# KubiakJakub01/Blokus-RL

Measured on AMD Instinct MI355X. Metric: MCTS sims/sec on 20x20 Blokus (4 players, 256 games/GPU, 100 sims/move), higher is better.
Workload: dtype fp32 net (fp32 operands split into f16 hi+lo, 3 f16 MFMA products, f32 accumulation: fp32-class error, tests/test_leafnet_gpu.py) / f64 search / u32 bitboards; 1 GPU; config 3 (N=1) / 4 (N=8): AlphaZero self-play 20x20, 256 concurrent games per GPU, 100 sims/move, ResNet-5x64 leaf eval; global_batch=256, parallelism=dp1 (independent games), model=resnet

## Files before the change

### blokus_rl_amd/csrc/leafnet.hip

```cpp
#include "../../include/blokus_engine.h"
#include "ctx.h"

#include <type_traits>

#define BK_LN_VACC 1
#include "leafnet_common.h"

#ifndef BK_LN_EPIW
#define BK_LN_EPIW 1
#endif

namespace bk {
namespace {

constexpr bool kLnEpiWrite = BK_LN_EPIW != 0;
#ifndef BK_LN_IL
#define BK_LN_IL 1
#endif
constexpr bool kLnInterleave = BK_LN_IL != 0;

struct LnStates {
  const uint32_t* states;
  const int32_t* status;
};
constexpr int kLnP = kStemCinX3 / 2;
constexpr int kLnRowWords = kLnP * kMaxN;

template <int N, typename In>
__global__ __launch_bounds__(kLnThreads, 1) void k_leafnet_x3(In in,
                                                              const h16x8* __restrict__ wstem_a,
                                                              const float* __restrict__ sstem_a,
                                                              const float* __restrict__ bstem_a,
                                                              const h16x8* __restrict__ wt_a,
                                                              const float* __restrict__ st_a,
                                                              const float* __restrict__ bt_a,
                                                              const float* __restrict__ bounds_a, int nlayers,
                                                              LnHeads hd_a, float* __restrict__ xout) {
  constexpr bool ROWS = std::is_same<In, LnRows>::value;
  constexpr bool STATES = std::is_same<In, LnStates>::value || ROWS;
  const h16x8* __restrict__ wstem = wstem_a;
  const float* __restrict__ sstem = sstem_a;
  const float* __restrict__ bstem = bstem_a;
  const h16x8* __restrict__ wt = wt_a;
  const float* __restrict__ st = st_a;
  const float* __restrict__ bt = bt_a;
  const float* __restrict__ bounds = bounds_a;
  LnHeads hd = hd_a;
  size_t b = blockIdx.x;
  if constexpr (ROWS) {
    int k;
    const int t = ln_row_tree(in, blockIdx.x, k);
    if (t < 0) return;
    b = (size_t)t;
    const LnNet nk = ln_pick(in.nets, k);
    wstem = nk.wstem;
    sstem = nk.sstem;
    bstem = nk.bstem;
    wt = nk.wt;
    st = nk.st;
    bt = nk.bt;
    bounds = nk.bounds;
    hd.wp = nk.wp;
    hd.bp = nk.bp;
    hd.wv = nk.wv;
    hd.bv = nk.bv;
    hd.w1t = nk.w1t;
    hd.b1 = nk.b1;
    hd.w2 = nk.w2;
    hd.b2 = nk.b2;
  }
  constexpr int NN = N * N, RS = ln_row(N), NG = ln_groups(N), PIX_IT = (NN + kLnThreads - 1) / kLnThreads;
  constexpr int PL = ln_plane(N);
  extern __shared__ __attribute__((aligned(16))) unsigned char lds[];
  unsigned char* act = lds;
  unsigned char* sin = lds + 16 * PL;
  float* red = reinterpret_cast<float*>(lds + ln_lds_body(N));
  constexpr int X0L = ln_x0_lds_groups(N);
  f32x4* x0s = reinterpret_cast<f32x4*>(lds + 16 * PL);
  const int tid = threadIdx.x, l = tid & 63, n = l & 15, ks = l >> 4;
  const int wave = __builtin_amdgcn_readfirstlane(tid >> 6);
  const int oc = 16 * wave + 4 * ks;
  LNSTAMP(0, __builtin_amdgcn_s_memtime());
  LNSTAMP(30, __builtin_amdgcn_s_memrealtime());

  float xin[STATES ? 1 : PIX_IT][kStemCinX3];
  uint32_t sw = 0u;
  bool live = true;
  if constexpr (STATES) {
    static_assert(kLnRowWords < kLnThreads && N <= kMaxN, "k_leafnet_x3: one state word per thread");
    live = ROWS || !in.status || in.status[b] == 1;
    if (live && tid <= kLnRowWords) sw = in.states[b * kStateWords + (tid < kLnRowWords ? tid : kWToMove)];
  } else {
    const float* __restrict__ ob = in + b * kStemCinX3 * NN;
#pragma unroll
    for (int it = 0; it < PIX_IT; ++it) {
      const int p = tid + it * kLnThreads;
#pragma unroll
      for (int c = 0; c < kStemCinX3; ++c) xin[it][c] = p < NN ? ob[c * NN + p] : 0.0f;
    }
  }
  {
    constexpr int kHaloCols = RS - N, kHalo = 2 * RS + N * kHaloCols;
    for (int i = tid; i < (STATES ? 17 : 18) * kHalo; i += kLnThreads) {
      const int plane = i / kHalo, k = i - plane * kHalo;
      int row, col;
      if (k < 2 * RS) {
        row = k < RS ? 0 : N + 1;
        col = k < RS ? k : k - RS;
      } else {
        const int h = k - 2 * RS, c = h % kHaloCols;
        row = 1 + h / kHaloCols;
        col = c == 0 ? 0 : N + c;
      }
      *reinterpret_cast<u32x4*>(lds + plane * PL + (row * RS + col) * 16) = u32x4{0u, 0u, 0u, 0u};
    }
  }

  constexpr int kBias = (RS + 1) * 16;
  int ab[NG];
  unsigned valid = 0;
#pragma unroll
  for (int g = 0; g < NG; ++g) {
    const int sl = kLnPixMap<N>.slot[16 * g + n];
    ab[g] = (sl >= 0 ? sl : RS + 1) * 16 + ks * 4 * PL - kBias;
    valid |= (sl >= 0 ? 1u : 0u) << g;
  }
  auto is_valid = [&](int g) { return NN % 16 == 0 || ((valid >> g) & 1u); };
  auto slot_b = [&](int g) { return ab[g] - ks * 4 * PL + kBias; };

  static_assert(18 % (kLnWpf + 1) == 0, "kLnWpf: the ring must divide the 18 chunks of a layer");
  constexpr int kLayerBlocks = 18 * 4 * 2;
  const __amdgpu_buffer_rsrc_t wrs = ln_rsrc(wt, (unsigned)nlayers * kLayerBlocks * 1024u);
  auto wload = [&](int layer, int c, int p) {
    return __builtin_bit_cast(h16x8, __builtin_amdgcn_raw_buffer_load_b128(
                                         wrs, l * 16, ((layer * kLayerBlocks + c * 8 + wave * 2 + p) * 64) * 16, 0));
  };
  h16x8 wq[kLnWpf + 1][2];
#pragma unroll
  for (int c = 0; c < kLnWpf; ++c) {
    wq[c][0] = wload(0, c, 0);
    wq[c][1] = wload(0, c, 1);
  }
  h16x8 wsa[3][2];
#pragma unroll
  for (int j = 0; j < 3; ++j) {
    wsa[j][0] = wstem[((j * 4 + wave) * 2) * 64 + l];
    wsa[j][1] = wstem[((j * 4 + wave) * 2 + 1) * 64 + l];
  }
  const f32x4 s_stem = *reinterpret_cast<const f32x4*>(sstem + oc), b_stem = *reinterpret_cast<const f32x4*>(bstem + oc);

  float max_obs;
  int ex;
  if constexpr (STATES) {
    uint32_t* rows = reinterpret_cast<uint32_t*>(sin + PL);
    bool any = false;
    if (tid < kLnRowWords) {
      const uint32_t bits = tid % kMaxN < N ? sw & ((1u << N) - 1u) : 0u;
      rows[tid] = bits;
      any = bits != 0u;
    } else if (tid == kLnRowWords) {
      const uint32_t tm = live ? sw : ~0u;
      rows[kLnRowWords] = tm;
      any = tm < (uint32_t)kLnP;
    }
    max_obs = block_max(any ? 1.0f : 0.0f, red + 8, wave, l);
    ex = scale_exp(max_obs);
    const unsigned one = __builtin_bit_cast(unsigned short, (_Float16)ldexpf(1.0f, ex));
    const uint32_t tm = rows[kLnRowWords];
    const unsigned m01 = ((tm == 0u ? 1u : 0u) | (tm == 1u ? 0x10000u : 0u)) * one;
    const unsigned m23 = ((tm == 2u ? 1u : 0u) | (tm == 3u ? 0x10000u : 0u)) * one;
#pragma unroll
    for (int it = 0; it < PIX_IT; ++it) {
      const int p = tid + it * kLnThreads;
      if (p < NN) {
        const int r = p / N, c = p % N;
        unsigned bit[kLnP];
#pragma unroll
        for (int q = 0; q < kLnP; ++q) bit[q] = (rows[q * kMaxN + r] >> c) & 1u;
        const u32x4 hi{(bit[0] | (bit[1] << 16)) * one, (bit[2] | (bit[3] << 16)) * one, m01, m23};
        *reinterpret_cast<u32x4*>(sin + ((r + 1) * RS + c + 1) * 16) = hi;
      }
    }
  } else {
    float m = 0.0f;
#pragma unroll
    for (int it = 0; it < PIX_IT; ++it)
#pragma unroll
      for (int c = 0; c < kStemCinX3; ++c) m = fmaxf(m, fabsf(xin[it][c]));
    max_obs = block_max(m, red + 8, wave, l);
    ex = scale_exp(max_obs);
#pragma unroll
    for (int it = 0; it < PIX_IT; ++it) {
      const int p = tid + it * kLnThreads;
      if (p < NN) {
        unsigned h[4], o[4];
#pragma unroll
        for (int q = 0; q < 4; ++q) split2(ldexpf(xin[it][2 * q], ex), ldexpf(xin[it][2 * q + 1], ex), h[q], o[q]);
        const u32x4 hi{h[0], h[1], h[2], h[3]}, lo{o[0], o[1], o[2], o[3]};
        unsigned char* dst = sin + ((p / N + 1) * RS + p % N + 1) * 16;
        *reinterpret_cast<u32x4*>(dst) = hi;
        *reinterpret_cast<u32x4*>(dst + PL) = lo;
      }
    }
  }
  __syncthreads();
  LNSTAMP(1, __builtin_amdgcn_s_memtime());
// ... 53 lines not shown
        split2(y01.x, y01.y, h0, l0);
        split2(y23.x, y23.y, h1, l1);
        if (write) {
          if (is_valid(g)) {
            *reinterpret_cast<u32x2*>(wbase + slot_b(g)) = u32x2{h0, h1};
            *reinterpret_cast<u32x2*>(wbase + slot_b(g) + PL) = u32x2{l0, l1};
          }
        } else {
          acc[g] = f32x4{__builtin_bit_cast(float, h0), __builtin_bit_cast(float, h1), __builtin_bit_cast(float, l0),
                         __builtin_bit_cast(float, l1)};
        }
      } else {
        acc[g] = f32x4{y01.x, y01.y, y23.x, y23.y};
      }
    }
    return ldexpf(mx, -k);
  };
  auto write_act = [&]() {
    const int o = 2 * wave + (ks >> 1);
    unsigned char* base = act + ((o & 3) * 4 + (o >> 2) * 2) * PL + (ks & 1) * 8;
#pragma unroll
    for (int g = 0; g < NG; ++g) {
      const u32x4 w = __builtin_bit_cast(u32x4, acc[g]);
      if (is_valid(g)) {
        *reinterpret_cast<u32x2*>(base + slot_b(g)) = u32x2{w.x, w.y};
        *reinterpret_cast<u32x2*>(base + slot_b(g) + PL) = u32x2{w.z, w.w};
      }
    }
  };
  auto out_exp = [&](int conv, float max_in) { return scale_exp(bounds[2 * conv] * max_in + bounds[2 * conv + 1]); };
  auto post_max = [&](float mx, int par) {
    mx = wave_max_f(mx);
    if (l == 0) red[4 * par + wave] = mx;
  };
  auto board_max = [&](int par) {
    return fmaxf(fmaxf(red[4 * par], red[4 * par + 1]), fmaxf(red[4 * par + 2], red[4 * par + 3]));
  };

  f32x4 x0[NG];
  float max_in;
  {
    const int ex_out = out_exp(0, max_obs);
#pragma unroll
    for (int g = 0; g < NG; ++g) x0[g] = f32x4{0.f, 0.f, 0.f, 0.f};
    const float mx = epilogue(s_stem, b_stem, true, false, x0, false, 0);
#pragma unroll
    for (int g = 0; g < NG; ++g) x0[g] = acc[g];
    const float up = ldexpf(1.0f, ex_out);
#pragma unroll
    for (int g = 0; g < NG; ++g) {
      unsigned h0, h1, l0, l1;
      split2(x0[g][0] * up, x0[g][1] * up, h0, l0);
      split2(x0[g][2] * up, x0[g][3] * up, h1, l1);
      acc[g] = f32x4{__builtin_bit_cast(float, h0), __builtin_bit_cast(float, h1), __builtin_bit_cast(float, l0),
                     __builtin_bit_cast(float, l1)};
    }
#pragma unroll
    for (int g = X0L; g < NG; ++g) asm volatile("" : "+a"(x0[g]));
    post_max(mx, 0);
    __syncthreads();
    write_act();
#pragma unroll
    for (int g = 0; g < X0L; ++g) {
      x0s[g * kLnThreads + tid] = x0[g];
      x0[g] = f32x4{0.f, 0.f, 0.f, 0.f};
    }
    __syncthreads();
    max_in = board_max(0);
    ex = ex_out;
  }
  LNSTAMP(3, __builtin_amdgcn_s_memtime());

  for (int layer = 0; layer < nlayers; ++layer) {
    const bool more = layer + 1 < nlayers;
    const f32x4 sv = *reinterpret_cast<const f32x4*>(st + layer * 64 + oc);
    const f32x4 bv = *reinterpret_cast<const f32x4*>(bt + layer * 64 + oc);
    const float bnd_a = bounds[2 * (layer + 1)], bnd_b = bounds[2 * (layer + 1) + 1];
    auto coff_of = [&](int c) {
      const int t = c >> 1;
      return 2 * (c & 1) * PL + ((t / 3 - 1) * RS + (t % 3 - 1)) * 16 + kBias;
    };
    ln_prime<NG, PL>(rb, act, ab, coff_of(0));
    if (layer == 1) LNSTAMP(26, __builtin_amdgcn_s_memtime());
#pragma unroll
    for (int c = 0; c < 18; ++c) {
      if (layer == 1 && c == 1) LNSTAMP(27, __builtin_amdgcn_s_memtime());
      if (layer == 1 && c == 9) LNSTAMP(28, __builtin_amdgcn_s_memtime());
      const int cn = c + kLnWpf, sn = cn % (kLnWpf + 1);
      if (cn < 18) {
        wq[sn][0] = wload(layer, cn, 0);
        wq[sn][1] = wload(layer, cn, 1);
      } else {
        const int nl = more ? layer + 1 : layer;
        wq[sn][0] = wload(nl, cn - 18, 0);
        wq[sn][1] = wload(nl, cn - 18, 1);
      }
      const h16x8* w = wq[c % (kLnWpf + 1)];
      if constexpr (kLnInterleave) {
        if (c == 0)
          ln_chunk_il<NG, true, PL>(acc, w[0], w[1], act, ab, coff_of(0), coff_of(1), rb);
        else
          ln_chunk_il<NG, false, PL>(acc, w[0], w[1], act, ab, coff_of(c), coff_of(c + 1 < 18 ? c + 1 : c), rb);
      } else {
        if (c == 0)
          ln_chunk<NG, true, PL>(acc, w[0], w[1], act, ab, coff_of(0), coff_of(1), rb);
        else
          ln_chunk<NG, false, PL>(acc, w[0], w[1], act, ab, coff_of(c), coff_of(c + 1 < 18 ? c + 1 : c), rb);
      }
    }
    if constexpr (kLnInterleave) asm volatile("s_waitcnt lgkmcnt(0)" ::: "memory");
    ln_mfma_drain(acc);
    if (layer < 8) LNSTAMP(4 + 2 * layer, __builtin_amdgcn_s_memtime());
    const bool last = layer + 1 == nlayers;
#ifndef BK_LN_ABL
#define BK_LN_ABL 0
#endif
    if (!last && BK_LN_ABL != 0) {
      if constexpr ((BK_LN_ABL & 2) == 0) {
        const int ex_out = scale_exp(bnd_a * max_in + bnd_b);
        const float mx = epilogue(sv, bv, !(layer & 1), false, x0, true, ex_out);
        max_in = fmaxf(max_in, mx);
        ex = ex_out;
      }
    } else if (!last && kLnEpiWrite) {
      const int ex_out = scale_exp(bnd_a * max_in + bnd_b);
      if (layer == 1) LNSTAMP(21, __builtin_amdgcn_s_memtime());
      __syncthreads();
      if (layer == 1) LNSTAMP(22, __builtin_amdgcn_s_memtime());
      const float mx = epilogue(sv, bv, !(layer & 1), false, x0, true, ex_out, true);
      if (layer == 1) LNSTAMP(23, __builtin_amdgcn_s_memtime());
      post_max(mx, (layer + 1) & 1);
      if (layer == 1) LNSTAMP(24, __builtin_amdgcn_s_memtime());
      __syncthreads();
      if (layer == 1) LNSTAMP(25, __builtin_amdgcn_s_memtime());
      max_in = board_max((layer + 1) & 1);
      ex = ex_out;
    } else if (!last) {
      const int ex_out = scale_exp(bnd_a * max_in + bnd_b);
      const float mx = epilogue(sv, bv, !(layer & 1), false, x0, true, ex_out);
      if (layer == 1) LNSTAMP(21, __builtin_amdgcn_s_memtime());
      post_max(mx, (layer + 1) & 1);
      if (layer == 1) LNSTAMP(22, __builtin_amdgcn_s_memtime());
      __syncthreads();
      if (layer == 1) LNSTAMP(23, __builtin_amdgcn_s_memtime());
      write_act();
      if (layer == 1) LNSTAMP(24, __builtin_amdgcn_s_memtime());
      __syncthreads();
      if (layer == 1) LNSTAMP(25, __builtin_amdgcn_s_memtime());
      max_in = board_max((layer + 1) & 1);
      ex = ex_out;
    } else {
#pragma unroll
      for (int g = 0; g < X0L; ++g) x0[g] = x0s[g * kLnThreads + tid];
      epilogue(sv, bv, true, true, x0, false, 0);
    }
    if (layer < 8) LNSTAMP(5 + 2 * layer, __builtin_amdgcn_s_memtime());
  }

  if (xout) {
#pragma unroll
    for (int g = 0; g < NG; ++g)
      if (is_valid(g))
        *reinterpret_cast<f32x4*>(xout + (b * NN + ln_pixel<N>(slot_b(g) / 16)) * 64 + oc) = acc[g];
  }
  __syncthreads();
  float* hp = reinterpret_cast<float*>(act);
  {
    const f32x4 wp0 = *reinterpret_cast<const f32x4*>(hd.wp + oc);
    const f32x4 wp1 = *reinterpret_cast<const f32x4*>(hd.wp + 64 + oc);
    const f32x4 wvv = *reinterpret_cast<const f32x4*>(hd.wv + oc);
#pragma unroll
    for (int g = 0; g < NG; ++g) {
      const f32x4 y = acc[g];
      float d[3];
      const f32x4* w[3] = {&wp0, &wp1, &wvv};
#pragma unroll
      for (int k = 0; k < 3; ++k) {
        const float a = y.x * (*w[k]).x + y.y * (*w[k]).y + y.z * (*w[k]).z + y.w * (*w[k]).w;
        const auto s16 = __builtin_amdgcn_permlane16_swap(__float_as_uint(a), __float_as_uint(a), false, false);
        const float a16 = __uint_as_float(s16[0]) + __uint_as_float(s16[1]);
        const auto s32 = __builtin_amdgcn_permlane32_swap(__float_as_uint(a16), __float_as_uint(a16), false, false);
        d[k] = __uint_as_float(s32[0]) + __uint_as_float(s32[1]);
      }
      if (ks == 0 && is_valid(g)) {
        float* dst = hp + (ln_pixel<N>(slot_b(g) / 16) * 4 + wave) * 3;
        dst[0] = d[0];
        dst[1] = d[1];
        dst[2] = d[2];
      }
    }
  }
  __syncthreads();
  LNSTAMP(20, __builtin_amdgcn_s_memtime());
  float* vfeat = hp + NN * 12;
  float* part = vfeat + NN;
  const float bp0 = hd.bp[0], bp1 = hd.bp[1], bv0 = hd.bv[0];
  for (int i = tid; i < NN; i += kLnThreads) {
    const float* q = hp + i * 12;
    const float p0 = ((q[0] + q[3]) + q[6]) + q[9], p1 = ((q[1] + q[4]) + q[7]) + q[10],
                pv = ((q[2] + q[5]) + q[8]) + q[11];
    hd.pf[b * 2 * NN + i] = fmaxf(p0 + bp0, 0.0f);
    hd.pf[b * 2 * NN + NN + i] = fmaxf(p1 + bp1, 0.0f);
    vfeat[i] = fmaxf(pv + bv0, 0.0f);
  }
  __syncthreads();
  {
    constexpr int Q = NN / 4;
    static_assert(NN % 4 == 0, "k_leafnet_x3: quarters of the value-MLP inputs");
    const int q0 = Q * wave;
    float w[Q];
#pragma unroll
    for (int k = 0; k < Q; ++k) w[k] = hd.w1t[(size_t)(q0 + k) * 64 + l];
    float a0 = 0.f, a1 = 0.f;
    int k = 0;
#pragma unroll
    for (; k + 10 <= Q; k += 10) {
#pragma unroll
      for (int u = 0; u < 10; u += 2) {
        a0 += w[k + u] * vfeat[q0 + k + u];
        a1 += w[k + u + 1] * vfeat[q0 + k + u + 1];
      }
    }
#pragma unroll
    for (; k < Q; ++k) a0 += w[k] * vfeat[q0 + k];
    part[wave * 64 + l] = a0 + a1;
  }
  __syncthreads();
  if (wave == 0) {
    float w2[kMaxP], b2[kMaxP];
#pragma unroll
    for (int q = 0; q < kMaxP; ++q) {
      w2[q] = q < hd.P ? hd.w2[q * 64 + l] : 0.0f;
      b2[q] = q < hd.P ? hd.b2[q] : 0.0f;
    }
    const float h = fmaxf(((part[l] + part[64 + l]) + (part[128 + l] + part[192 + l])) + hd.b1[l], 0.0f);
#pragma unroll
    for (int q = 0; q < kMaxP; ++q) {
      if (q < hd.P) {
        const float sum = wave_sum_f(w2[q] * h);
        if (l == 0) hd.v[b * hd.P + q] = tanhf(sum + b2[q]);
      }
    }
  }
  LNSTAMP(29, __builtin_amdgcn_s_memtime());
  LNSTAMP(31, __builtin_amdgcn_s_memrealtime());
}

static_assert(ln_lds_bytes(20) <= 160 * 1024, "k_leafnet_x3<20>: LDS");

}
}

using namespace bk;

extern "C" {

int bk_leafnet_x3_weight_bytes(int cin) {
  return cin == 64 || cin == 8 ? ln_chunks(cin) * 4 * 2 * kBlock * 2 : -1;
}

int bk_leafnet_x3_supported(int N) { return N == 14 || N == 20; }

#if BK_LN_STAMP
int bk_ln_stamps(unsigned long long* out) {
  return hipMemcpyFromSymbol(out, HIP_SYMBOL(g_ln_stamps), sizeof(g_ln_stamps)) == hipSuccess ? 0 : -1;
}
int bk_ln_stamps_clear() {
  static unsigned long long zeros[256 * 4 * kLnStamps];
  return hipMemcpyToSymbol(HIP_SYMBOL(g_ln_stamps), zeros, sizeof(zeros)) == hipSuccess ? 0 : -1;
}
#endif

int bk_leafnet_x3(const float* obs, int B, int N, int cin, const void* wstem, const float* sstem, const float* bstem,
                  int nlayers, const void* wtower, const float* stower, const float* btower, const float* bounds,
                  const float* wp,
                  const float* bp, const float* wv, const float* bv, const float* w1t, const float* b1,
                  const float* w2, const float* b2, int P, float* pf, float* vout, float* out, void* stream) {
  BK_REQUIRE(obs && wstem && sstem && bstem && wtower && stower && btower && bounds && B >= 0, "bad argument");
  BK_REQUIRE(wp && bp && wv && bv && w1t && b1 && w2 && b2 && pf && vout && P > 0, "bad argument");
  BK_REQUIRE(cin == kStemCinX3, "bk_leafnet_x3: the stem takes 8 observation planes");
  BK_REQUIRE(nlayers >= 1, "bk_leafnet_x3: at least one tower conv");
  BK_REQUIRE(bk_leafnet_x3_supported(N), "bk_leafnet_x3: N must be 14 or 20");
  const auto a16 = [](const void* p) { return ((uintptr_t)p & 15u) == 0; };
  BK_REQUIRE(a16(wstem) && a16(wtower) && a16(sstem) && a16(bstem) && a16(stower) && a16(btower) && a16(wp) &&
                 a16(wv) && a16(out),
             "bk_leafnet_x3: 16-byte aligned buffers");
  if (B == 0) return BK_OK;
  {
    const void* fns[2] = {(const void*)k_leafnet_x3<14, const float*>, (const void*)k_leafnet_x3<20, const float*>};
    if (set_max_dynamic_lds(fns, 2, ln_lds_bytes(20)) != BK_OK) return BK_EHIP;
  }
  const LnHeads h{wp, bp, wv, bv, w1t, b1, w2, b2, P, pf, vout};
  hipStream_t s = (hipStream_t)stream;
  const h16x8* ws = reinterpret_cast<const h16x8*>(wstem);
  const h16x8* wt = reinterpret_cast<const h16x8*>(wtower);
  if (N == 20)
    hipLaunchKernelGGL((k_leafnet_x3<20, const float*>), dim3(B), dim3(kLnThreads), ln_lds_bytes(20), s, obs, ws, sstem,
                       bstem, wt, stower, btower, bounds, nlayers, h, out);
  else
    hipLaunchKernelGGL((k_leafnet_x3<14, const float*>), dim3(B), dim3(kLnThreads), ln_lds_bytes(14), s, obs, ws, sstem,
                       bstem, wt, stower, btower, bounds, nlayers, h, out);
  return launch_check("k_leafnet_x3");
}

int bk_leafnet_x3_states(const void* states, const int32_t* status, int B, int N, int P, const void* wstem,
                         const float* sstem, const float* bstem, int nlayers, const void* wtower,
                         const float* stower, const float* btower, const float* bounds, const float* wp,
                         const float* bp, const float* wv, const float* bv, const float* w1t, const float* b1,
                         const float* w2, const float* b2, float* pf, float* vout, float* out, void* stream) {
  BK_REQUIRE(states && wstem && sstem && bstem && wtower && stower && btower && bounds && B >= 0, "bad argument");
  BK_REQUIRE(wp && bp && wv && bv && w1t && b1 && w2 && b2 && pf && vout, "bad argument");
  BK_REQUIRE(P == kLnP, "bk_leafnet_x3_states: P must be 4 (the stem takes 8 observation planes)");
  BK_REQUIRE(nlayers >= 1, "bk_leafnet_x3_states: at least one tower conv");
  BK_REQUIRE(bk_leafnet_x3_supported(N), "bk_leafnet_x3_states: N must be 14 or 20");
  BK_REQUIRE(((uintptr_t)states & 3u) == 0, "bk_leafnet_x3_states: states must be 4-byte aligned");
  const auto a16 = [](const void* p) { return ((uintptr_t)p & 15u) == 0; };
  BK_REQUIRE(a16(wstem) && a16(wtower) && a16(sstem) && a16(bstem) && a16(stower) && a16(btower) && a16(wp) &&
                 a16(wv) && a16(out),
             "bk_leafnet_x3_states: 16-byte aligned buffers");
  if (B == 0) return BK_OK;
  {
    const void* fns[2] = {(const void*)k_leafnet_x3<14, LnStates>, (const void*)k_leafnet_x3<20, LnStates>};
    if (set_max_dynamic_lds(fns, 2, ln_lds_bytes(20)) != BK_OK) return BK_EHIP;
  }
  const LnHeads h{wp, bp, wv, bv, w1t, b1, w2, b2, P, pf, vout};
  hipStream_t s = (hipStream_t)stream;
  const h16x8* ws = reinterpret_cast<const h16x8*>(wstem);
  const h16x8* wt = reinterpret_cast<const h16x8*>(wtower);
  const LnStates in{reinterpret_cast<const uint32_t*>(states), status};
  if (N == 20)
    hipLaunchKernelGGL((k_leafnet_x3<20, LnStates>), dim3(B), dim3(kLnThreads), ln_lds_bytes(20), s, in, ws, sstem, bstem,
                       wt, stower, btower, bounds, nlayers, h, out);
  else
    hipLaunchKernelGGL((k_leafnet_x3<14, LnStates>), dim3(B), dim3(kLnThreads), ln_lds_bytes(14), s, in, ws, sstem, bstem,
                       wt, stower, btower, bounds, nlayers, h, out);
  return launch_check("k_leafnet_x3 (states)");
}

int bk_leafnet_x3_rows(const bk_leafnet_args* nets, int nnets, const bk_arena_rows* rows, int sim, void* stream) {
  BK_REQUIRE(rows && nnets >= 0 && nnets <= kLnMaxNets && sim >= 0, "bk_leafnet_x3_rows: bad argument");
  BK_REQUIRE(rows->R >= 0 && rows->T >= 0 && (rows->R == 0 || (rows->tree_of_row && rows->net_of_row && rows->sims_of_row)),
             "bk_leafnet_x3_rows: bad row tables");
  if (nnets == 0 || rows->R == 0) return BK_OK;
  BK_REQUIRE(nets, "bk_leafnet_x3_rows: null net table");
  const bk_leafnet_args& a0 = nets[0];
  const auto a16 = [](const void* p) { return ((uintptr_t)p & 15u) == 0; };
  for (int k = 0; k < nnets; ++k) {
    const bk_leafnet_args& a = nets[k];
    BK_REQUIRE(!a.obs && a.states && a.status, "bk_leafnet_x3_rows: states form only (states and status set, obs null)");
    BK_REQUIRE(a.states == a0.states && a.status == a0.status && a.pf == a0.pf && a.vout == a0.vout && a.N == a0.N &&
                   a.P == a0.P && a.nlayers == a0.nlayers && a.np == a0.np,
               "bk_leafnet_x3_rows: the nets must share states, status, pf, vout, N, P, nlayers and np");
    BK_REQUIRE(a.wstem && a.sstem && a.bstem && a.wtower && a.stower && a.btower && a.bounds && a.wp && a.bp && a.wv &&
                   a.bv && a.w1t && a.b1 && a.w2 && a.b2 && a.pf && a.vout,
               "bk_leafnet_x3_rows: null net operand");
    BK_REQUIRE(a16(a.wstem) && a16(a.wtower) && a16(a.sstem) && a16(a.bstem) && a16(a.stower) && a16(a.btower) &&
                   a16(a.wp) && a16(a.wv),
               "bk_leafnet_x3_rows: 16-byte aligned buffers");
  }
  BK_REQUIRE(a0.nlayers >= 1, "bk_leafnet_x3_rows: at least one tower conv");
  BK_REQUIRE(((uintptr_t)a0.states & 3u) == 0, "bk_leafnet_x3_rows: states must be 4-byte aligned");
  if (a0.np) return bk::leafnet_np_rows(nets, nnets, rows, sim, stream);
  BK_REQUIRE(a0.P == kLnP, "bk_leafnet_x3_rows: the classic form takes P = 4 (np = 0)");
  BK_REQUIRE(bk_leafnet_x3_supported(a0.N), "bk_leafnet_x3_rows: N must be 14 or 20 (np = 0)");
  {
    const void* fns[2] = {(const void*)k_leafnet_x3<14, LnRows>, (const void*)k_leafnet_x3<20, LnRows>};
    if (set_max_dynamic_lds(fns, 2, ln_lds_bytes(20)) != BK_OK) return BK_EHIP;
  }
  const LnRows in = ln_rows_of(nets, nnets, rows, sim);
  const LnHeads h{nullptr, nullptr, nullptr, nullptr, nullptr, nullptr, nullptr, nullptr, a0.P, a0.pf, a0.vout};
  hipStream_t s = (hipStream_t)stream;
  const h16x8* nw = nullptr;
  const float* nf = nullptr;
  float* out = nullptr;
  if (a0.N == 20)
    hipLaunchKernelGGL((k_leafnet_x3<20, LnRows>), dim3(rows->R), dim3(kLnThreads), ln_lds_bytes(20), s, in, nw, nf, nf,
                       nw, nf, nf, nf, a0.nlayers, h, out);
  else
    hipLaunchKernelGGL((k_leafnet_x3<14, LnRows>), dim3(rows->R), dim3(kLnThreads), ln_lds_bytes(14), s, in, nw, nf, nf,
                       nw, nf, nf, nf, a0.nlayers, h, out);
  return launch_check("k_leafnet_x3 (rows)");
}

}
```

### blokus_rl_amd/csrc/leafnet_common.h

```cpp
#pragma once
#include "../../include/blokus_engine.h"
#include "ctx.h"

namespace bk {
int leafnet_np_rows(const bk_leafnet_args* nets, int nnets, const bk_arena_rows* rows, int sim, void* stream);

namespace {

using h16x8 = _Float16 __attribute__((ext_vector_type(8)));
using h16x2 = _Float16 __attribute__((ext_vector_type(2)));
using f32x4 = float __attribute__((ext_vector_type(4)));
using f32x2 = float __attribute__((ext_vector_type(2)));
using u32x4 = unsigned __attribute__((ext_vector_type(4)));
using u32x2 = unsigned __attribute__((ext_vector_type(2)));

#ifndef BK_LN_DUMMY
#define BK_LN_DUMMY 0
#endif
#ifndef BK_LN_STAMP
#define BK_LN_STAMP 0
#endif
#if BK_LN_STAMP
constexpr int kLnStamps = 32;
__device__ unsigned long long g_ln_stamps[256 * 4 * kLnStamps];
#define LNSTAMP(i, v)                                                                                          \
  do {                                                                                                         \
    if (l == 0 && blockIdx.x < 256) g_ln_stamps[(blockIdx.x * 4 + wave) * kLnStamps + (i)] = (v);              \
  } while (0)
#else
#define LNSTAMP(i, v) \
  do {                \
  } while (0)
#endif

constexpr int kLnThreads = 256;
constexpr int kStemCinX3 = 8;
constexpr int kBlock = 64 * 8;

__host__ __device__ constexpr int ln_chunks(int cin) { return cin == 64 ? 18 : 3; }

#ifndef BK_LN_VACC
#define BK_LN_VACC 0
#endif
#if BK_LN_VACC
#define BK_ACC_W "=&v"
#define BK_ACC_RW "+v"
#else
#define BK_ACC_W "=&a"
#define BK_ACC_RW "+a"
#endif
constexpr int kLnPf = 2, kLnSlots = 5, kLnWpf = 1;
static_assert(kLnPf >= 1 && kLnPf < kLnSlots, "kLnPf");
__host__ __device__ constexpr int ln_groups(int N) { return ((N * N + 15) / 16 + kLnSlots - 1) / kLnSlots * kLnSlots; }

__host__ __device__ constexpr int ln_row(int N) { return N == 14 ? 18 : N + 2; }
__host__ __device__ constexpr int ln_plane(int N) { return ((N + 2) * ln_row(N) * 16 + 255) / 256 * 256; }
__host__ __device__ constexpr int ln_x0_lds_groups(int N) { return N == 20 ? 7 : 0; }
__host__ __device__ constexpr int ln_lds_body(int N) {
  return 16 * ln_plane(N) + (2 * ln_plane(N) > ln_x0_lds_groups(N) * 256 * 16 ? 2 * ln_plane(N)
                                                                                 : ln_x0_lds_groups(N) * 256 * 16);
}
__host__ __device__ constexpr int ln_lds_bytes(int N) { return ln_lds_body(N) + 64; }

template <int N>
struct LnPixMap {
  static constexpr int NN = N * N, NG = ln_groups(N), RS = ln_row(N);
  int slot[NG * 16];
  constexpr LnPixMap() : slot() {
    bool used[NN] = {};
    for (int i = 0; i < NG * 16; ++i) slot[i] = -1;
    for (int g = 0; g < NG; ++g)
      for (int r = 0; r < 16; ++r)
        for (int p = 0; p < NN; ++p) {
          const int sl = (p / N + 1) * RS + p % N + 1;
          if (!used[p] && sl % 16 == r) {
            used[p] = true;
            slot[g * 16 + r] = sl;
            break;
          }
        }
    int p = 0;
    for (int i = 0; i < NG * 16; ++i) {
      if (slot[i] >= 0) continue;
      while (p < NN && used[p]) ++p;
      if (p == NN) break;
      used[p] = true;
      slot[i] = (p / N + 1) * RS + p % N + 1;
    }
  }
};
template <int N>
__device__ constexpr LnPixMap<N> kLnPixMap{};
template <int N>
__device__ __forceinline__ int ln_pixel(int slot) {
  return (slot / ln_row(N) - 1) * N + slot % ln_row(N) - 1;
}

__device__ __forceinline__ f32x4 mfma16(h16x8 a, h16x8 b, f32x4 c) {
  return __builtin_amdgcn_mfma_f32_16x16x32_f16(a, b, c, 0, 0, 0);
}

__device__ __forceinline__ void split2(float x0, float x1, unsigned& hi, unsigned& lo) {
  asm("v_cvt_pk_f16_f32 %0, %2, %3\n\t"
      "v_fma_mixlo_f16 %1, -%0, 1.0, %2 op_sel_hi:[1,0,0]\n\t"
      "v_fma_mixhi_f16 %1, -%0, 1.0, %3 op_sel:[1,0,0] op_sel_hi:[1,0,0]"
      : "=&v"(hi), "=&v"(lo)
      : "v"(x0), "v"(x1));
}

__device__ __forceinline__ f32x2 pk_fma(f32x2 a, f32x2 b, f32x2 c) {
  f32x2 r;
  asm("v_pk_fma_f32 %0, %1, %2, %3" : "=v"(r) : "v"(a), "v"(b), "v"(c));
  return r;
}
__device__ __forceinline__ f32x2 pk_add(f32x2 a, f32x2 b) {
  f32x2 r;
  asm("v_pk_add_f32 %0, %1, %2" : "=v"(r) : "v"(a), "v"(b));
  return r;
}

__device__ __forceinline__ f32x2 pk_sub(f32x2 a, f32x2 b) {
  f32x2 r;
  asm("v_pk_add_f32 %0, %1, %2 neg_lo:[0,1] neg_hi:[0,1]" : "=v"(r) : "v"(a), "v"(b));
  return r;
}
__device__ __forceinline__ f32x4 add4(f32x4 a, f32x4 b) {
  const f32x2 lo = pk_add(f32x2{a.x, a.y}, f32x2{b.x, b.y}), hi = pk_add(f32x2{a.z, a.w}, f32x2{b.z, b.w});
  return f32x4{lo.x, lo.y, hi.x, hi.y};
}
__device__ __forceinline__ f32x4 sub4(f32x4 a, f32x4 b) {
  const f32x2 lo = pk_sub(f32x2{a.x, a.y}, f32x2{b.x, b.y}), hi = pk_sub(f32x2{a.z, a.w}, f32x2{b.z, b.w});
  return f32x4{lo.x, lo.y, hi.x, hi.y};
}
__device__ __forceinline__ f32x4 fma4(f32x4 a, f32x4 b, f32x4 c) {
  const f32x2 lo = pk_fma(f32x2{a.x, a.y}, f32x2{b.x, b.y}, f32x2{c.x, c.y});
  const f32x2 hi = pk_fma(f32x2{a.z, a.w}, f32x2{b.z, b.w}, f32x2{c.z, c.w});
  return f32x4{lo.x, lo.y, hi.x, hi.y};
}

__device__ __forceinline__ float max3_abs(float m, float a, float b) {
  float r;
  asm("v_max3_f32 %0, %1, |%2|, |%3|" : "=v"(r) : "v"(m), "v"(a), "v"(b));
  return r;
}
__device__ __forceinline__ float max_bits(float y, int floor) {
  return __builtin_bit_cast(float, max(__builtin_bit_cast(int, y), floor));
}

__device__ __forceinline__ __amdgpu_buffer_rsrc_t ln_rsrc(const void* p, unsigned bytes) {
  const uintptr_t a = (uintptr_t)p;
  const uintptr_t u = ((uintptr_t)(unsigned)__builtin_amdgcn_readfirstlane((int)(a >> 32)) << 32) |
                      (unsigned)__builtin_amdgcn_readfirstlane((int)(unsigned)a);
  return __builtin_amdgcn_make_buffer_rsrc((void*)u, 0, (int)bytes, 0x00020000);
}

__device__ __forceinline__ int scale_exp(float m) {
  if (!(m > 0.0f) || !(m < __builtin_inff())) return 0;
  int e;
  (void)frexpf(m, &e);
  const int s = 15 - e;
  return s < -64 ? -64 : (s > 64 ? 64 : s);
}

__device__ __forceinline__ float block_max(float m, float* red, int wave, int l) {
  m = wave_max_f(m);
  if (l == 0) red[wave] = m;
  __syncthreads();
  return fmaxf(fmaxf(red[0], red[1]), fmaxf(red[2], red[3]));
}

template <int HALF>
__device__ __forceinline__ void ln_load(h16x8 (&r)[2], const unsigned char* grid, int pb, int coff) {
  const unsigned char* q = grid + pb + coff;
  r[0] = *reinterpret_cast<const h16x8*>(q);
  r[1] = *reinterpret_cast<const h16x8*>(q + HALF);
// ... 57 lines not shown
template <int NG, bool INIT>
__device__ __forceinline__ void ln_chunk_hi(f32x4 (&acc)[NG], h16x8 ah, h16x8 al, const unsigned char* grid,
                                            const int (&pb)[NG], int coff, int coff_next, h16x8 (&rb)[kLnSlots][2]) {
  static_assert(NG % kLnSlots == 0, "ln_chunk_hi: the ring slot of a group must not depend on the chunk");
#pragma unroll
  for (int g = 0; g < NG; ++g) {
    const int gp = g + kLnPf;
    rb[gp % kLnSlots][0] = *reinterpret_cast<const h16x8*>(grid + (gp < NG ? pb[gp] + coff : pb[gp - NG] + coff_next));
    const h16x8 bh = rb[g % kLnSlots][0];
    if (INIT)
      asm volatile(
          "v_mfma_f32_16x16x32_f16 %0, %1, %2, 0\n\t"
          "v_mfma_f32_16x16x32_f16 %0, %3, %2, %0"
          : BK_ACC_W(acc[g])
          : "v"(ah), "v"(bh), "v"(al));
    else
      asm volatile(
          "v_mfma_f32_16x16x32_f16 %0, %1, %2, %0\n\t"
          "v_mfma_f32_16x16x32_f16 %0, %3, %2, %0"
          : BK_ACC_RW(acc[g])
          : "v"(ah), "v"(bh), "v"(al));
  }
}

template <int NG, bool INIT, int HALF>
__device__ __forceinline__ void ln_chunk_il(f32x4 (&acc)[NG], h16x8 ah, h16x8 al, const unsigned char* grid,
                                            const int (&pb)[NG], int coff, int coff_next, h16x8 (&rb)[kLnSlots][2]) {
  static_assert(NG % kLnSlots == 0, "ln_chunk_il: the ring slot of a group must not depend on the chunk");
  const unsigned gbase = (unsigned)(uintptr_t)grid;
#pragma unroll
  for (int g = 0; g < NG; ++g) {
    const int gp = g + kLnPf;
    const unsigned addr = gbase + (unsigned)(gp < NG ? pb[gp] : pb[gp - NG]);
    h16x8& n0 = rb[gp % kLnSlots][0];
    h16x8& n1 = rb[gp % kLnSlots][1];
    if (gp < NG) {
      if (INIT)
        asm volatile(
            "s_waitcnt lgkmcnt(%10)\n\t"
            "v_mfma_f32_16x16x32_f16 %0, %3, %5, 0\n\t"
            "ds_read_b128 %1, %7 offset:%8\n\t"
            "v_mfma_f32_16x16x32_f16 %0, %4, %5, %0\n\t"
            "ds_read_b128 %2, %7 offset:%9\n\t"
            "v_mfma_f32_16x16x32_f16 %0, %3, %6, %0"
            : BK_ACC_W(acc[g]), "=&v"(n0), "=&v"(n1)
            : "v"(ah), "v"(al), "v"(rb[g % kLnSlots][0]), "v"(rb[g % kLnSlots][1]), "v"(addr), "i"(coff), "i"(coff + HALF), "i"(2 * (kLnPf - 1)));
      else
        asm volatile(
            "s_waitcnt lgkmcnt(%10)\n\t"
            "v_mfma_f32_16x16x32_f16 %0, %3, %5, %0\n\t"
            "ds_read_b128 %1, %7 offset:%8\n\t"
            "v_mfma_f32_16x16x32_f16 %0, %4, %5, %0\n\t"
            "ds_read_b128 %2, %7 offset:%9\n\t"
            "v_mfma_f32_16x16x32_f16 %0, %3, %6, %0"
            : BK_ACC_RW(acc[g]), "=&v"(n0), "=&v"(n1)
            : "v"(ah), "v"(al), "v"(rb[g % kLnSlots][0]), "v"(rb[g % kLnSlots][1]), "v"(addr), "i"(coff), "i"(coff + HALF), "i"(2 * (kLnPf - 1)));
    } else {
      if (INIT)
        asm volatile(
            "s_waitcnt lgkmcnt(%10)\n\t"
            "v_mfma_f32_16x16x32_f16 %0, %3, %5, 0\n\t"
            "ds_read_b128 %1, %7 offset:%8\n\t"
            "v_mfma_f32_16x16x32_f16 %0, %4, %5, %0\n\t"
            "ds_read_b128 %2, %7 offset:%9\n\t"
            "v_mfma_f32_16x16x32_f16 %0, %3, %6, %0"
            : BK_ACC_W(acc[g]), "=&v"(n0), "=&v"(n1)
            : "v"(ah), "v"(al), "v"(rb[g % kLnSlots][0]), "v"(rb[g % kLnSlots][1]), "v"(addr), "i"(coff_next),
              "i"(coff_next + HALF), "i"(2 * (kLnPf - 1)));
      else
        asm volatile(
            "s_waitcnt lgkmcnt(%10)\n\t"
            "v_mfma_f32_16x16x32_f16 %0, %3, %5, %0\n\t"
            "ds_read_b128 %1, %7 offset:%8\n\t"
            "v_mfma_f32_16x16x32_f16 %0, %4, %5, %0\n\t"
            "ds_read_b128 %2, %7 offset:%9\n\t"
            "v_mfma_f32_16x16x32_f16 %0, %3, %6, %0"
            : BK_ACC_RW(acc[g]), "=&v"(n0), "=&v"(n1)
            : "v"(ah), "v"(al), "v"(rb[g % kLnSlots][0]), "v"(rb[g % kLnSlots][1]), "v"(addr), "i"(coff_next),
              "i"(coff_next + HALF), "i"(2 * (kLnPf - 1)));
    }
  }
}

template <int NG>
__device__ __forceinline__ void ln_mfma_drain(f32x4 (&acc)[NG]) {
  asm volatile("s_nop 7\n\ts_nop 7\n\ts_nop 7" ::: "memory");
#pragma unroll
  for (int g = 0; g < NG; ++g) asm volatile("" : BK_ACC_RW(acc[g]));
}

struct LnHeads {
  const float *wp, *bp, *wv, *bv, *w1t, *b1, *w2, *b2;
  int P;
  float* pf;
  float* v;
};

constexpr int kLnMaxNets = BK_ARENA_MAX_NETS;
struct LnNet {
  const h16x8* wstem;
  const float *sstem, *bstem;
  const h16x8* wt;
  const float *st, *bt, *bounds;
  const float *wp, *bp, *wv, *bv, *w1t, *b1, *w2, *b2;
};
struct LnRows {
  const uint32_t* states;
  const int32_t* status;
  const int32_t *tree, *net, *sims;
  int sim, nnets, ntrees;
  LnNet nets[kLnMaxNets];
};
__device__ __forceinline__ LnNet ln_pick(const LnNet (&n)[kLnMaxNets], int k) {
  LnNet o;
#define BK_LN_PICK(f) o.f = k == 0 ? n[0].f : k == 1 ? n[1].f : k == 2 ? n[2].f : n[3].f
  BK_LN_PICK(wstem);
  BK_LN_PICK(sstem);
  BK_LN_PICK(bstem);
  BK_LN_PICK(wt);
  BK_LN_PICK(st);
  BK_LN_PICK(bt);
  BK_LN_PICK(bounds);
  BK_LN_PICK(wp);
  BK_LN_PICK(bp);
  BK_LN_PICK(wv);
  BK_LN_PICK(bv);
  BK_LN_PICK(w1t);
  BK_LN_PICK(b1);
  BK_LN_PICK(w2);
  BK_LN_PICK(b2);
#undef BK_LN_PICK
  return o;
}
inline LnRows ln_rows_of(const bk_leafnet_args* nets, int nnets, const bk_arena_rows* rows, int sim) {
  LnRows in{};
  in.states = reinterpret_cast<const uint32_t*>(nets[0].states);
  in.status = nets[0].status;
  in.tree = rows->tree_of_row;
  in.net = rows->net_of_row;
  in.sims = rows->sims_of_row;
  in.sim = sim;
  in.nnets = nnets;
  in.ntrees = rows->T;
  for (int k = 0; k < nnets; ++k) {
    const bk_leafnet_args& a = nets[k];
    in.nets[k] = LnNet{reinterpret_cast<const h16x8*>(a.wstem), a.sstem, a.bstem,
                       reinterpret_cast<const h16x8*>(a.wtower), a.stower, a.btower, a.bounds,
                       a.wp, a.bp, a.wv, a.bv, a.w1t, a.b1, a.w2, a.b2};
  }
  return in;
}
__device__ __forceinline__ int ln_row_tree(const LnRows& in, int r, int& k) {
  const int t = __builtin_amdgcn_readfirstlane(in.tree[r]);
  k = -1;
  if (t < 0 || t >= in.ntrees || in.sim >= __builtin_amdgcn_readfirstlane(in.sims[r])) return -1;
  k = __builtin_amdgcn_readfirstlane(in.net[r]);
  if (k < 0 || k >= in.nnets) return -1;
  return __builtin_amdgcn_readfirstlane(in.status[t]) == 1 ? t : -1;
}

}
}
```

Baseline: 1.376 million sims/s.

## Skip MFMA work on board-edge pixel groups whose 3x3 taps read only halo

Adds an alternate pixel-to-MFMA-column map for the 20x20 board that packs the four edge strips into dedicated groups. A compile-time schedule then drops the conv chunks where those groups would read only zero halo, removing 24 of 450 group-chunk MFMA triples per layer. The LDS read ring is re-sequenced per chunk to match the variable active groups. The path is on by default and can be disabled with BK_LN_EDGE; it adds a third kernel instantiation and more complex compile-time scheduling.

```diff
diff --git a/blokus_rl_amd/csrc/leafnet.hip b/blokus_rl_amd/csrc/leafnet.hip
--- a/blokus_rl_amd/csrc/leafnet.hip
+++ b/blokus_rl_amd/csrc/leafnet.hip
@@ -26,7 +26,7 @@
 constexpr int kLnP = kStemCinX3 / 2;
 constexpr int kLnRowWords = kLnP * kMaxN;
 
-template <int N, typename In>
+template <int N, typename In, bool EDGE_A = false>
 __global__ __launch_bounds__(kLnThreads, 1) void k_leafnet_x3(In in,
                                                               const h16x8* __restrict__ wstem_a,
                                                               const float* __restrict__ sstem_a,
@@ -38,6 +38,7 @@
                                                               LnHeads hd_a, float* __restrict__ xout) {
   constexpr bool ROWS = std::is_same<In, LnRows>::value;
   constexpr bool STATES = std::is_same<In, LnStates>::value || ROWS;
+  constexpr bool EDGE = EDGE_A && kLnInterleave;
   const h16x8* __restrict__ wstem = wstem_a;
   const float* __restrict__ sstem = sstem_a;
   const float* __restrict__ bstem = bstem_a;
@@ -121,7 +122,11 @@
   unsigned valid = 0;
 #pragma unroll
   for (int g = 0; g < NG; ++g) {
-    const int sl = kLnPixMap<N>.slot[16 * g + n];
+    int sl;
+    if constexpr (EDGE)
+      sl = kLnEdgePixMap<N>.slot[16 * g + n];
+    else
+      sl = kLnPixMap<N>.slot[16 * g + n];
     ab[g] = (sl >= 0 ? sl : RS + 1) * 16 + ks * 4 * PL - kBias;
     valid |= (sl >= 0 ? 1u : 0u) << g;
   }
@@ -341,30 +346,47 @@
     };
     ln_prime<NG, PL>(rb, act, ab, coff_of(0));
     if (layer == 1) LNSTAMP(26, __builtin_amdgcn_s_memtime());
-#pragma unroll
-    for (int c = 0; c < 18; ++c) {
-      if (layer == 1 && c == 1) LNSTAMP(27, __builtin_amdgcn_s_memtime());
-      if (layer == 1 && c == 9) LNSTAMP(28, __builtin_amdgcn_s_memtime());
-      const int cn = c + kLnWpf, sn = cn % (kLnWpf + 1);
-      if (cn < 18) {
-        wq[sn][0] = wload(layer, cn, 0);
-        wq[sn][1] = wload(layer, cn, 1);
-      } else {
-        const int nl = more ? layer + 1 : layer;
-        wq[sn][0] = wload(nl, cn - 18, 0);
-        wq[sn][1] = wload(nl, cn - 18, 1);
-      }
-      const h16x8* w = wq[c % (kLnWpf + 1)];
-      if constexpr (kLnInterleave) {
-        if (c == 0)
-          ln_chunk_il<NG, true, PL>(acc, w[0], w[1], act, ab, coff_of(0), coff_of(1), rb);
-        else
-          ln_chunk_il<NG, false, PL>(acc, w[0], w[1], act, ab, coff_of(c), coff_of(c + 1 < 18 ? c + 1 : c), rb);
-      } else {
-        if (c == 0)
-          ln_chunk<NG, true, PL>(acc, w[0], w[1], act, ab, coff_of(0), coff_of(1), rb);
-        else
-          ln_chunk<NG, false, PL>(acc, w[0], w[1], act, ab, coff_of(c), coff_of(c + 1 < 18 ? c + 1 : c), rb);
+    if constexpr (EDGE) {
+      ln_each_chunk(
+          [&](auto cc) __attribute__((always_inline)) {
+            constexpr int c = decltype(cc)::value, cn = c + kLnWpf, sn = cn % (kLnWpf + 1);
+            using S = LnEdgeSched<N>;
+            if (layer == 1 && c == 1) LNSTAMP(27, __builtin_amdgcn_s_memtime());
+            if (layer == 1 && c == 9) LNSTAMP(28, __builtin_amdgcn_s_memtime());
+            const int wl = cn < 18 || more ? layer + cn / 18 : layer;
+            wq[sn][0] = wload(wl, cn % 18, 0);
+            wq[sn][1] = wload(wl, cn % 18, 1);
+            const h16x8* w = wq[c % (kLnWpf + 1)];
+            ln_chunk_il_act<NG, S::active(c), S::first(c), S::pos0(c), PL>(acc, w[0], w[1], act, ab, coff_of(c),
+                                                                         coff_of(c + 1 < 18 ? c + 1 : c), rb);
+          },
+          std::make_integer_sequence<int, 18>{});
+    } else {
+#pragma unroll
+      for (int c = 0; c < 18; ++c) {
+        if (layer == 1 && c == 1) LNSTAMP(27, __builtin_amdgcn_s_memtime());
+        if (layer == 1 && c == 9) LNSTAMP(28, __builtin_amdgcn_s_memtime());
+        const int cn = c + kLnWpf, sn = cn % (kLnWpf + 1);
+        if (cn < 18) {
+          wq[sn][0] = wload(layer, cn, 0);
+          wq[sn][1] = wload(layer, cn, 1);
+        } else {
+          const int nl = more ? layer + 1 : layer;
+          wq[sn][0] = wload(nl, cn - 18, 0);
+          wq[sn][1] = wload(nl, cn - 18, 1);
+        }
+        const h16x8* w = wq[c % (kLnWpf + 1)];
+        if constexpr (kLnInterleave) {
+          if (c == 0)
+            ln_chunk_il<NG, true, PL>(acc, w[0], w[1], act, ab, coff_of(0), coff_of(1), rb);
+          else
+            ln_chunk_il<NG, false, PL>(acc, w[0], w[1], act, ab, coff_of(c), coff_of(c + 1 < 18 ? c + 1 : c), rb);
+        } else {
+          if (c == 0)
+            ln_chunk<NG, true, PL>(acc, w[0], w[1], act, ab, coff_of(0), coff_of(1), rb);
+          else
+            ln_chunk<NG, false, PL>(acc, w[0], w[1], act, ab, coff_of(c), coff_of(c + 1 < 18 ? c + 1 : c), rb);
+        }
       }
     }
     if constexpr (kLnInterleave) asm volatile("s_waitcnt lgkmcnt(0)" ::: "memory");
@@ -506,6 +528,14 @@
 }
 
 static_assert(ln_lds_bytes(20) <= 160 * 1024, "k_leafnet_x3<20>: LDS");
+static_assert(ln_edge_map_is_bijection<20>(), "LnEdgePixMap<20>: every board pixel in exactly one MFMA column");
+static_assert(ln_edge_sched_skips_only_halo<20>(), "LnEdgeSched<20>: a skipped (group, chunk) reads only the halo");
+static_assert(LnEdgeSched<20>::pos0(18) == 18 * 25 - 24, "LnEdgeSched<20>: 24 of 450 pairs left out");
+
+bool ln_edge() {
+  const char* e = getenv("BK_LN_EDGE");
+  return e ? atoi(e) != 0 : true;
+}
 
 }
 }
@@ -546,14 +576,18 @@
              "bk_leafnet_x3: 16-byte aligned buffers");
   if (B == 0) return BK_OK;
   {
-    const void* fns[2] = {(const void*)k_leafnet_x3<14, const float*>, (const void*)k_leafnet_x3<20, const float*>};
-    if (set_max_dynamic_lds(fns, 2, ln_lds_bytes(20)) != BK_OK) return BK_EHIP;
+    const void* fns[3] = {(const void*)k_leafnet_x3<14, const float*>, (const void*)k_leafnet_x3<20, const float*>,
+                          (const void*)k_leafnet_x3<20, const float*, true>};
+    if (set_max_dynamic_lds(fns, 3, ln_lds_bytes(20)) != BK_OK) return BK_EHIP;
   }
   const LnHeads h{wp, bp, wv, bv, w1t, b1, w2, b2, P, pf, vout};
   hipStream_t s = (hipStream_t)stream;
   const h16x8* ws = reinterpret_cast<const h16x8*>(wstem);
   const h16x8* wt = reinterpret_cast<const h16x8*>(wtower);
-  if (N == 20)
+  if (N == 20 && ln_edge())
+    hipLaunchKernelGGL((k_leafnet_x3<20, const float*, true>), dim3(B), dim3(kLnThreads), ln_lds_bytes(20), s, obs, ws,
+                       sstem, bstem, wt, stower, btower, bounds, nlayers, h, out);
+  else if (N == 20)
     hipLaunchKernelGGL((k_leafnet_x3<20, const float*>), dim3(B), dim3(kLnThreads), ln_lds_bytes(20), s, obs, ws, sstem,
                        bstem, wt, stower, btower, bounds, nlayers, h, out);
   else
@@ -579,15 +613,19 @@
              "bk_leafnet_x3_states: 16-byte aligned buffers");
   if (B == 0) return BK_OK;
   {
-    const void* fns[2] = {(const void*)k_leafnet_x3<14, LnStates>, (const void*)k_leafnet_x3<20, LnStates>};
-    if (set_max_dynamic_lds(fns, 2, ln_lds_bytes(20)) != BK_OK) return BK_EHIP;
+    const void* fns[3] = {(const void*)k_leafnet_x3<14, LnStates>, (const void*)k_leafnet_x3<20, LnStates>,
+                          (const void*)k_leafnet_x3<20, LnStates, true>};
+    if (set_max_dynamic_lds(fns, 3, ln_lds_bytes(20)) != BK_OK) return BK_EHIP;
   }
   const LnHeads h{wp, bp, wv, bv, w1t, b1, w2, b2, P, pf, vout};
   hipStream_t s = (hipStream_t)stream;
   const h16x8* ws = reinterpret_cast<const h16x8*>(wstem);
   const h16x8* wt = reinterpret_cast<const h16x8*>(wtower);
   const LnStates in{reinterpret_cast<const uint32_t*>(states), status};
-  if (N == 20)
+  if (N == 20 && ln_edge())
+    hipLaunchKernelGGL((k_leafnet_x3<20, LnStates, true>), dim3(B), dim3(kLnThreads), ln_lds_bytes(20), s, in, ws, sstem,
+                       bstem, wt, stower, btower, bounds, nlayers, h, out);
+  else if (N == 20)
     hipLaunchKernelGGL((k_leafnet_x3<20, LnStates>), dim3(B), dim3(kLnThreads), ln_lds_bytes(20), s, in, ws, sstem, bstem,
                        wt, stower, btower, bounds, nlayers, h, out);
   else
@@ -623,8 +661,9 @@
   BK_REQUIRE(a0.P == kLnP, "bk_leafnet_x3_rows: the classic form takes P = 4 (np = 0)");
   BK_REQUIRE(bk_leafnet_x3_supported(a0.N), "bk_leafnet_x3_rows: N must be 14 or 20 (np = 0)");
   {
-    const void* fns[2] = {(const void*)k_leafnet_x3<14, LnRows>, (const void*)k_leafnet_x3<20, LnRows>};
-    if (set_max_dynamic_lds(fns, 2, ln_lds_bytes(20)) != BK_OK) return BK_EHIP;
+    const void* fns[3] = {(const void*)k_leafnet_x3<14, LnRows>, (const void*)k_leafnet_x3<20, LnRows>,
+                          (const void*)k_leafnet_x3<20, LnRows, true>};
+    if (set_max_dynamic_lds(fns, 3, ln_lds_bytes(20)) != BK_OK) return BK_EHIP;
   }
   const LnRows in = ln_rows_of(nets, nnets, rows, sim);
   const LnHeads h{nullptr, nullptr, nullptr, nullptr, nullptr, nullptr, nullptr, nullptr, a0.P, a0.pf, a0.vout};
@@ -632,7 +671,10 @@
   const h16x8* nw = nullptr;
   const float* nf = nullptr;
   float* out = nullptr;
-  if (a0.N == 20)
+  if (a0.N == 20 && ln_edge())
+    hipLaunchKernelGGL((k_leafnet_x3<20, LnRows, true>), dim3(rows->R), dim3(kLnThreads), ln_lds_bytes(20), s, in, nw, nf,
+                       nf, nw, nf, nf, nf, a0.nlayers, h, out);
+  else if (a0.N == 20)
     hipLaunchKernelGGL((k_leafnet_x3<20, LnRows>), dim3(rows->R), dim3(kLnThreads), ln_lds_bytes(20), s, in, nw, nf, nf,
                        nw, nf, nf, nf, a0.nlayers, h, out);
   else
diff --git a/blokus_rl_amd/csrc/leafnet_common.h b/blokus_rl_amd/csrc/leafnet_common.h
--- a/blokus_rl_amd/csrc/leafnet_common.h
+++ b/blokus_rl_amd/csrc/leafnet_common.h
@@ -1,6 +1,9 @@
 #pragma once
 #include "../../include/blokus_engine.h"
 #include "ctx.h"
+
+#include <type_traits>
+#include <utility>
 
 namespace bk {
 int leafnet_np_rows(const bk_leafnet_args* nets, int nnets, const bk_arena_rows* rows, int sim, void* stream);
@@ -91,6 +94,106 @@
 };
 template <int N>
 __device__ constexpr LnPixMap<N> kLnPixMap{};
+
+template <int N>
+struct LnEdgePixMap {
+  static constexpr int NN = N * N, NG = ln_groups(N), RS = ln_row(N), G0 = NG - 4;
+  static_assert(N == 20 && NG * 16 == NN, "LnEdgePixMap: the 20x20 board (no spare columns)");
+  static constexpr int edge_pixel(int e, int i) {
+    return e == 0 ? 2 + i : e == 1 ? (N - 1) * N + 2 + i : e == 2 ? (2 + i) * N : (2 + i) * N + N - 1;
+  }
+  int slot[NG * 16];
+  constexpr LnEdgePixMap() : slot() {
+    bool used[NN] = {};
+    for (int i = 0; i < NG * 16; ++i) slot[i] = -1;
+    for (int e = 0; e < 4; ++e)
+      for (int i = 0; i < 16; ++i) {
+        const int p = edge_pixel(e, i);
+        used[p] = true;
+        slot[(G0 + e) * 16 + i] = (p / N + 1) * RS + p % N + 1;
+      }
+    for (int g = 0; g < G0; ++g)
+      for (int r = 0; r < 16; ++r)
+        for (int p = 0; p < NN; ++p) {
+          const int sl = (p / N + 1) * RS + p % N + 1;
+          if (!used[p] && sl % 16 == r) {
+            used[p] = true;
+            slot[g * 16 + r] = sl;
+            break;
+          }
+        }
+    int p = 0;
+    for (int i = 0; i < G0 * 16; ++i) {
+      if (slot[i] >= 0) continue;
+      while (p < NN && used[p]) ++p;
+      if (p == NN) break;
+      used[p] = true;
+      slot[i] = (p / N + 1) * RS + p % N + 1;
+    }
+  }
+};
+template <int N>
+__device__ constexpr LnEdgePixMap<N> kLnEdgePixMap{};
+
+template <int N>
+struct LnEdgeSched {
+  static constexpr int NG = ln_groups(N), G0 = NG - 4, NC = ln_chunks(64);
+  static constexpr bool skips(int g, int c) {
+    const int t = c >> 1, dy = t / 3 - 1, dx = t % 3 - 1;
+    return g == G0 ? dy < 0 : g == G0 + 1 ? dy > 0 : g == G0 + 2 ? dx < 0 : g == G0 + 3 ? dx > 0 : false;
+  }
+  static constexpr unsigned active(int c) {
+    unsigned m = 0;
+    for (int g = 0; g < NG; ++g) m |= (skips(g, c) ? 0u : 1u) << g;
+    return m;
+  }
+  static constexpr unsigned first(int c) {
+    unsigned m = active(c);
+    for (int k = 0; k < c; ++k) m &= ~active(k);
+    return m;
+  }
+  static constexpr int pos0(int c) {
+    int n = 0;
+    for (int k = 0; k < c; ++k)
+      for (int g = 0; g < NG; ++g) n += skips(g, k) ? 0 : 1;
+    return n;
+  }
+};
+template <int N>
+constexpr bool ln_edge_map_is_bijection() {
+  constexpr int RS = ln_row(N), NG = ln_groups(N);
+  const LnEdgePixMap<N> m{};
+  bool seen[N * N] = {};
+  for (int i = 0; i < NG * 16; ++i) {
+    const int sl = m.slot[i];
+    if (sl < 0) return false;
+    const int r = sl / RS - 1, c = sl % RS - 1;
+    if (r < 0 || r >= N || c < 0 || c >= N || seen[r * N + c]) return false;
+    seen[r * N + c] = true;
+  }
+  return true;
+}
+template <int N>
+constexpr bool ln_edge_sched_skips_only_halo() {
+  using S = LnEdgeSched<N>;
+  constexpr int RS = ln_row(N);
+  const LnEdgePixMap<N> m{};
+  unsigned ran = 0;
+  for (int c = 0; c < S::NC; ++c) {
+    const int t = c >> 1, dy = t / 3 - 1, dx = t % 3 - 1;
+    if ((S::active(c) & ((1u << kLnPf) - 1u)) != (1u << kLnPf) - 1u) return false;
+    ran |= S::active(c);
+    for (int g = 0; g < S::NG; ++g) {
+      if (!S::skips(g, c)) continue;
+      for (int n = 0; n < 16; ++n) {
+        const int sl = m.slot[g * 16 + n], r = sl / RS - 1 + dy, col = sl % RS - 1 + dx;
+        if (r >= 0 && r < N && col >= 0 && col < N) return false;
+      }
+    }
+  }
+  return ran == (1u << S::NG) - 1u;
+}
+
 template <int N>
 __device__ __forceinline__ int ln_pixel(int slot) {
   return (slot / ln_row(N) - 1) * N + slot % ln_row(N) - 1;
@@ -314,6 +417,84 @@
   }
 }
 
+template <int NG, unsigned ACT>
+struct LnActive {
+  int n;
+  int g[NG + kLnPf];
+  constexpr LnActive() : n(0), g() {
+    for (int k = 0; k < NG; ++k)
+      if ((ACT >> k) & 1u) g[n++] = k;
+    for (int k = 0; k < kLnPf; ++k) g[n + k] = NG + k;
+  }
+};
+
+template <int NG, unsigned ACT, unsigned INIT, int POS0, int HALF>
+__device__ __forceinline__ void ln_chunk_il_act(f32x4 (&acc)[NG], h16x8 ah, h16x8 al, const unsigned char* grid,
+                                                const int (&pb)[NG], int coff, int coff_next,
+                                                h16x8 (&rb)[kLnSlots][2]) {
+  constexpr LnActive<NG, ACT> A{};
+  static_assert((INIT & ~ACT) == 0u && A.n >= kLnPf, "ln_chunk_il_act: INIT groups run; the ring fits the chunk");
+  const unsigned gbase = (unsigned)(uintptr_t)grid;
+#pragma unroll
+  for (int i = 0; i < A.n; ++i) {
+    const int g = A.g[i], gp = A.g[i + kLnPf];
+    const int s = (POS0 + i) % kLnSlots, sp = (POS0 + i + kLnPf) % kLnSlots;
+    const unsigned addr = gbase + (unsigned)(gp < NG ? pb[gp] : pb[gp - NG]);
+    h16x8& n0 = rb[sp][0];
+    h16x8& n1 = rb[sp][1];
+    if (gp < NG) {
+      if ((INIT >> g) & 1u)
+        asm volatile(
+            "s_waitcnt lgkmcnt(%10)\n\t"
+            "v_mfma_f32_16x16x32_f16 %0, %3, %5, 0\n\t"
+            "ds_read_b128 %1, %7 offset:%8\n\t"
+            "v_mfma_f32_16x16x32_f16 %0, %4, %5, %0\n\t"
+            "ds_read_b128 %2, %7 offset:%9\n\t"
+            "v_mfma_f32_16x16x32_f16 %0, %3, %6, %0"
+            : BK_ACC_W(acc[g]), "=&v"(n0), "=&v"(n1)
+            : "v"(ah), "v"(al), "v"(rb[s][0]), "v"(rb[s][1]), "v"(addr), "i"(coff), "i"(coff + HALF), "i"(2 * (kLnPf - 1)));
+      else
+        asm volatile(
+            "s_waitcnt lgkmcnt(%10)\n\t"
+            "v_mfma_f32_16x16x32_f16 %0, %3, %5, %0\n\t"
+            "ds_read_b128 %1, %7 offset:%8\n\t"
+            "v_mfma_f32_16x16x32_f16 %0, %4, %5, %0\n\t"
+            "ds_read_b128 %2, %7 offset:%9\n\t"
+            "v_mfma_f32_16x16x32_f16 %0, %3, %6, %0"
+            : BK_ACC_RW(acc[g]), "=&v"(n0), "=&v"(n1)
+            : "v"(ah), "v"(al), "v"(rb[s][0]), "v"(rb[s][1]), "v"(addr), "i"(coff), "i"(coff + HALF), "i"(2 * (kLnPf - 1)));
+    } else {
+      if ((INIT >> g) & 1u)
+        asm volatile(
+            "s_waitcnt lgkmcnt(%10)\n\t"
+            "v_mfma_f32_16x16x32_f16 %0, %3, %5, 0\n\t"
+            "ds_read_b128 %1, %7 offset:%8\n\t"
+            "v_mfma_f32_16x16x32_f16 %0, %4, %5, %0\n\t"
+            "ds_read_b128 %2, %7 offset:%9\n\t"
+            "v_mfma_f32_16x16x32_f16 %0, %3, %6, %0"
+            : BK_ACC_W(acc[g]), "=&v"(n0), "=&v"(n1)
+            : "v"(ah), "v"(al), "v"(rb[s][0]), "v"(rb[s][1]), "v"(addr), "i"(coff_next), "i"(coff_next + HALF),
+              "i"(2 * (kLnPf - 1)));
+      else
+        asm volatile(
+            "s_waitcnt lgkmcnt(%10)\n\t"
+            "v_mfma_f32_16x16x32_f16 %0, %3, %5, %0\n\t"
+            "ds_read_b128 %1, %7 offset:%8\n\t"
+            "v_mfma_f32_16x16x32_f16 %0, %4, %5, %0\n\t"
+            "ds_read_b128 %2, %7 offset:%9\n\t"
+            "v_mfma_f32_16x16x32_f16 %0, %3, %6, %0"
+            : BK_ACC_RW(acc[g]), "=&v"(n0), "=&v"(n1)
+            : "v"(ah), "v"(al), "v"(rb[s][0]), "v"(rb[s][1]), "v"(addr), "i"(coff_next), "i"(coff_next + HALF),
+              "i"(2 * (kLnPf - 1)));
+    }
+  }
+}
+
+template <class F, int... Cs>
+__device__ __forceinline__ void ln_each_chunk(F&& f, std::integer_sequence<int, Cs...>) {
+  (f(std::integral_constant<int, Cs>{}), ...);
+}
+
 template <int NG>
 __device__ __forceinline__ void ln_mfma_drain(f32x4 (&acc)[NG]) {
   asm volatile("s_nop 7\n\ts_nop 7\n\ts_nop 7" ::: "memory");
```

Measured after the change: 1.417 million sims/s, median of 6. +3.0%, better.
